# Wang-Xiaoyang/resource_packing_self_play

Hardware: AMD Instinct MI355X
Metric: self-play episodes/sec (with MCTS node expansions/sec alongside) (higher is better)
Workload: dtype f64 PUCT / f32 Q + CNN, u32 bit-board

## Files before the change

### resource_packing_self_play_amd/csrc/rp_engine.hip

```cpp
#include <hip/hip_runtime.h>
#include <math.h>
#include <stdarg.h>
#include <stdint.h>
#include <stdio.h>
#include <stdlib.h>
#include <string.h>

#include <algorithm>
#include <string>
#include <vector>

#include "../../include/rp_engine.h"

#pragma clang fp contract(off)

typedef unsigned long long u64;
typedef unsigned int u32;
typedef unsigned short u16;
typedef unsigned char u8;

#define NONE32 0xFFFFFFFFu
#define NSA_MASK 0x3FFFFFFFu
#define WAVES_PER_BLOCK 4
#define MAX_LEAVES 128
#define MAX_MASK_WORDS 256

enum { CNT_SIMS = 0, CNT_EXPAND, CNT_TERMINAL, CNT_PATH, CNT_NVALID_SEL, CNT_NVALID_LEAF, CNT_TRANSPOSE, CNT_NODES,
       CNT_MOVES, CNT_EPISODES, CNT_PROBES, CNT_KEYBYTES, CNT_VIS_SEL, CNT_VIS_NEW, CNT_RES0, CNT_RES1, CNT_N };
enum { ERR_NODE_CAP = 1, ERR_EDGE_CAP = 2, ERR_TABLE_FULL = 3, ERR_BAD_ACTION = 4, ERR_PATH = 5, ERR_FINISHED_CAP = 6, ERR_EXAMPLES_CAP = 7, ERR_VIS_CAP = 8, ERR_BAD_EXAMPLE = 9 };

struct NodeHdr {
    u32 ns;
    u32 prior_off;
    u32 vis_off;
    u16 n_valid;
    u16 vis_n;
    u16 vis_cap;
    int8_t term;
    u8 flags;
    u8 depth;
    u8 pad;
    u16 best_k;
    double norm;
};
#define HF_EXPANDED 1u
#define HF_FALLBACK 2u
__host__ __device__ inline u32 hdr_term_kind(const NodeHdr &h) { return (h.flags >> 2) & 3u; }

struct PoolDesc {
    long long n_instances;
    unsigned long long first_id;
    const unsigned char *wh;
    const int *area, *max_h;
    const unsigned long long *episode_id;
    const double *bl;
    const unsigned char *has_buf;
};
struct VisEntry {
    double q;
    double p;
    u32 n;
    u32 child;
    u32 idx;
    u32 pad;
};
struct DP {
    int W, H, N, A, G, sims, node_cap, edge_cap, vis_cap, table_cap, KW, RW, RMW, move_rule;
    int reclaim;
    int pchunk, n_pchunks, vchunk, n_vchunks;
    int step_cap;
    u32 magicW;
    double cpuct;
    u64 seed, tie_salt;
    u8 *item_wh;
    int *total_area, *max_h;
    double *bl;
    int *has_buf;
    u32 *root, *n_nodes;
    u16 *pa_cur, *pa_head, *pa_next, *pa_stack, *va_cur, *va_head, *va_next, *va_stack;
    u32 *pa_used, *pa_tf, *va_used, *va_tf;
    u32 *peak_chunks;
    int *phase, *sims_done, *moves;
    u64 *episode;
    u32 *leaf_node;
    int *path_len;
    u32 *path_edge, *path_node;
    int *game_row;
    int *last_outcome;
    double *last_score;
    double *last_v;
    int *last_vkind;
    int rows_identity;
// ... 2383 lines not shown
    for (int t = 0; t < NT; ++t) {
        const int m = t * 16 + n, pc = m < MP ? ptab[m] : IMGW * IMGP;
        abase[t] = (ptab[m < MP ? m : 0] - (PW + 1)) * PS + 8 * g;
        pdst[t][0] = pc * PS + 4 * g;
        pdst[t][1] = pc * PS + 16 + 4 * g;
    }
    const __amdgpu_buffer_rsrc_t frs = __builtin_amdgcn_make_buffer_rsrc((void *)frag, 0, 4 * 9 * CIN * 32 * 4, RS_BUF_FLAGS);
    constexpr int CONV_BYTES = 9 * CIN * 32 * 4;
    const int rowoff = n * 128 + g * 16;
    auto task_bytes = [&](long long l0) { return (int)(B - l0 < IMGW ? B - l0 : IMGW) * PIX * 128; };
    f32x4 xv[NT][2], xs[NT][2], wq[3][2];
    auto load_x = [&](long long l0) {
        const __amdgpu_buffer_rsrc_t rs = __builtin_amdgcn_make_buffer_rsrc((void *)(x + (size_t)l0 * PIX * CIN), 0, task_bytes(l0), RS_BUF_FLAGS);
#pragma unroll
        for (int t = 0; t < NT; ++t) { xv[t][0] = rs_load_x(rs, rowoff, t * 2048); xv[t][1] = rs_load_x(rs, rowoff, t * 2048 + 64); }
    };
    auto stage_x = [&]() {
#pragma unroll
        for (int t = 0; t < NT; ++t)
#pragma unroll
            for (int mt = 0; mt < 2; ++mt) { xs[t][mt] = xv[t][mt]; *(f32x4 *)(img + pdst[t][mt]) = rs_relu(xv[t][mt]); }
    };
    load_x(leaf0);
    wq[0][0] = rs_load_b(frs, lane * 16, 0); wq[0][1] = rs_load_b(frs, lane * 16, 1024);
    wq[1][0] = rs_load_b(frs, lane * 16, 2048); wq[1][1] = rs_load_b(frs, lane * 16, 3072);
    stage_x();
    if (leaf0 + stride_leaves < B) load_x(leaf0 + stride_leaves);
    for (; leaf0 < B; leaf0 += stride_leaves) {
        const int nbytes = task_bytes(leaf0);
        const __amdgpu_buffer_rsrc_t ors = __builtin_amdgcn_make_buffer_rsrc((void *)(out + (size_t)leaf0 * PIX * CIN), 0, nbytes, RS_BUF_FLAGS);
        f32x4 acc[NT][2];
#define R32_BIAS(k) const f32x4 ba = *(const f32x4 *)(sbias + 32 * (k) + 4 * g), bb = *(const f32x4 *)(sbias + 32 * (k) + 16 + 4 * g)
        lds_sync();
        r32_conv<NT, CIN>(img, frs, 0, CONV_BYTES, PW, abase, acc, wq);
        {
            R32_BIAS(0);
#pragma unroll
            for (int t = 0; t < NT; ++t) { *(f32x4 *)(img + pdst[t][0]) = rs_relu(acc[t][0] + ba); *(f32x4 *)(img + pdst[t][1]) = rs_relu(acc[t][1] + bb); }
        }
        lds_sync();
        r32_conv<NT, CIN>(img, frs, CONV_BYTES, 2 * CONV_BYTES, PW, abase, acc, wq);
        {
            R32_BIAS(1);
#pragma unroll
            for (int t = 0; t < NT; ++t) {
                xs[t][0] = (acc[t][0] + ba) + xs[t][0]; xs[t][1] = (acc[t][1] + bb) + xs[t][1];
                *(f32x4 *)(img + pdst[t][0]) = rs_relu(xs[t][0]); *(f32x4 *)(img + pdst[t][1]) = rs_relu(xs[t][1]);
            }
        }
        lds_sync();
        r32_conv<NT, CIN>(img, frs, 2 * CONV_BYTES, 3 * CONV_BYTES, PW, abase, acc, wq);
        {
            R32_BIAS(2);
#pragma unroll
            for (int t = 0; t < NT; ++t) { *(f32x4 *)(img + pdst[t][0]) = rs_relu(acc[t][0] + ba); *(f32x4 *)(img + pdst[t][1]) = rs_relu(acc[t][1] + bb); }
        }
        lds_sync();
        r32_conv<NT, CIN>(img, frs, 3 * CONV_BYTES, 0, PW, abase, acc, wq);
        {
            R32_BIAS(3);
#pragma unroll
            for (int t = 0; t < NT; ++t) {
                acc[t][0] = (acc[t][0] + ba) + xs[t][0]; acc[t][1] = (acc[t][1] + bb) + xs[t][1];
                __builtin_amdgcn_raw_buffer_store_b128(__builtin_bit_cast(u32x4, acc[t][0]), ors, rowoff, t * 2048, RS_STREAM_AUX);
                __builtin_amdgcn_raw_buffer_store_b128(__builtin_bit_cast(u32x4, acc[t][1]), ors, rowoff, t * 2048 + 64, RS_STREAM_AUX);
            }
        }
#undef R32_BIAS
        if (out_relu != nullptr) {
            const __amdgpu_buffer_rsrc_t rrs = __builtin_amdgcn_make_buffer_rsrc((void *)(out_relu + (size_t)leaf0 * PIX * CIN), 0, nbytes, RS_BUF_FLAGS);
#pragma unroll
            for (int t = 0; t < NT; ++t) {
                __builtin_amdgcn_raw_buffer_store_b128(__builtin_bit_cast(u32x4, rs_relu(acc[t][0])), rrs, rowoff, t * 2048, RS_STREAM_AUX);
                __builtin_amdgcn_raw_buffer_store_b128(__builtin_bit_cast(u32x4, rs_relu(acc[t][1])), rrs, rowoff, t * 2048 + 64, RS_STREAM_AUX);
            }
        }
        if (leaf0 + stride_leaves < B) {
            stage_x();
            if (leaf0 + 2 * stride_leaves < B) load_x(leaf0 + 2 * stride_leaves);
        }
    }
}

#define CP_PS 36
#ifdef CP_STAMP
__device__ unsigned long long g_cp_stamp[8];
#endif
template <int NT, int CIN, bool TAIL = false>
__global__ void __launch_bounds__(256, 2) k_convpool32(const float *__restrict__ x, const float *__restrict__ frag, const float *__restrict__ bias,
                                                       float *__restrict__ out, long long B, int S_h, int S_w, int IMGW, int wave_floats,
                                                       const int *__restrict__ nrows_dev) {
    constexpr int XQ = CIN / 16;
    constexpr int PS = CP_PS;
    extern __shared__ __attribute__((aligned(16))) float rb_lds[];
    const int lane = lane_id(), wv = wave_in_block();
    if (nrows_dev) { const long long n = *nrows_dev; if (n < B) B = n; }
    if (((long long)blockIdx.x * 4) * IMGW >= B) return;
    const int PW = r32_pw(S_w), PIX = S_h * S_w, IMGP = r32_imgp(S_h, S_w), MP = IMGW * PIX;
    const int Hp = (S_h + 1) >> 1, Wp = (S_w + 1) >> 1, PP = Hp * Wp;
    constexpr int NTT = NT + (TAIL ? 1 : 0);
    int *ptab = (int *)rb_lds;
    int *pool = ptab + 16 * NTT;
    float *img = rb_lds + 16 * NTT + ((IMGW * PP + 3) & ~3) + (size_t)wv * wave_floats;
    for (int i = threadIdx.x; i < 16 * NTT; i += blockDim.x) {
        int im = i / PIX, pq = i - im * PIX, r = pq / S_w, c = pq - r * S_w;
        ptab[i] = i < MP ? im * IMGP + (r + 1) * PW + c + 1 : 0;
    }
    for (int i = threadIdx.x; i < IMGW * PP; i += blockDim.x) {
        int im = i / PP, pp = i - im * PP, pr = pp / Wp, px = pp - pr * Wp;
        pool[i] = (im * IMGP + (2 * pr + 1) * PW + 2 * px + 1) | ((pr > 0) << 16) | ((2 * pr + 1 < S_h) << 17) | ((px > 0) << 18) | ((2 * px + 1 < S_w) << 19);
    }
    {
        float4 *z4 = (float4 *)img;
        for (int i = lane; i < wave_floats / 4; i += 64) z4[i] = make_float4(0.f, 0.f, 0.f, 0.f);
    }
    __syncthreads();
    const long long stride_leaves = (long long)gridDim.x * 4 * IMGW;
    long long leaf0 = ((long long)blockIdx.x * 4 + wv) * IMGW;
    if (leaf0 >= B) return;
    const int n = lane & 15, g = lane >> 4;
    int abase[NT], pin[NT];
#pragma unroll
    for (int t = 0; t < NT; ++t) {
        const int m = t * 16 + n, pc = m < MP ? ptab[m] : IMGW * IMGP;
        abase[t] = (ptab[m < MP ? m : 0] - (PW + 1)) * PS + CIN / 4 * g;
        pin[t] = pc * PS + 4 * g;
    }
    const __amdgpu_buffer_rsrc_t frs = __builtin_amdgcn_make_buffer_rsrc((void *)frag, 0, 9 * CIN * 32 * 4, RS_BUF_FLAGS);
    const f32x4 ba = *(const f32x4 *)(bias + 4 * g), bb = *(const f32x4 *)(bias + 16 + 4 * g);
    const int rowoff = n * (CIN * 4) + g * 16;
    auto task_bytes = [&](long long l0) { return (int)(B - l0 < IMGW ? B - l0 : IMGW) * PIX * CIN * 4; };
    f32x4 xv[NT][XQ], wq[3][2];
    int t_abase = 0, t_voff0 = 0, t_voff1 = 0;
    f32x4 t_acc = (f32x4){0.f, 0.f, 0.f, 0.f}, t_w0[2], t_w1[2];
    const int cg = lane >> 3, kk = (lane >> 2) & 1, mt = 16 * NT + (lane & 3);
    int pout_t = 0, pin_t = 0;
    f32x4 xvt = (f32x4){0.f, 0.f, 0.f, 0.f};
    const int xq_t = (lane >> 2) & (CIN / 4 - 1);
    const int rowoff_t = (lane & 3) * (CIN * 4) + xq_t * 16;
    if (TAIL) {
        const int pc = mt < MP ? ptab[mt] : IMGW * IMGP;
        t_abase = (ptab[mt < MP ? mt : 0] - (PW + 1)) * PS + (CIN / 2) * kk;
        const int lw = 4 * (cg & 3) + (lane & 3) + 32 * kk;
        t_voff0 = (cg >> 2) * 1024 + lw * 16; t_voff1 = (cg >> 2) * 1024 + (lw + 16) * 16;
        pout_t = pc * PS + 4 * cg;
        pin_t = pc * PS + 4 * xq_t;
    }
    auto load_x = [&](long long l0) {
        const __amdgpu_buffer_rsrc_t rs = __builtin_amdgcn_make_buffer_rsrc((void *)(x + (size_t)l0 * PIX * CIN), 0, task_bytes(l0), RS_BUF_FLAGS);
#pragma unroll
        for (int t = 0; t < NT; ++t)
#pragma unroll
            for (int q = 0; q < XQ; ++q) xv[t][q] = rs_load_x(rs, rowoff, t * 16 * CIN * 4 + 64 * q);
        if (TAIL) xvt = rs_load_x(rs, rowoff_t, NT * 16 * CIN * 4);
    };
    const int cq = lane & 7;
    load_x(leaf0);
    wq[0][0] = rs_load_b(frs, lane * 16, 0); wq[0][1] = rs_load_b(frs, lane * 16, 1024);
    wq[1][0] = rs_load_b(frs, lane * 16, 2048); wq[1][1] = rs_load_b(frs, lane * 16, 3072);
    if (TAIL) {
        t_w0[0] = rs_load_b(frs, t_voff0, 0); t_w1[0] = rs_load_b(frs, t_voff1, 0);
        t_w0[1] = rs_load_b(frs, t_voff0, 2048); t_w1[1] = rs_load_b(frs, t_voff1, 2048);
    }
#ifdef CP_STAMP
    unsigned long long st_acc[8] = {0, 0, 0, 0, 0, 0, 0, 0}, st_last = __builtin_amdgcn_s_memtime();
#define CP_T(k) { unsigned long long now_ = __builtin_amdgcn_s_memtime(); st_acc[k] += now_ - st_last; st_last = now_; }
// ... 289 lines not shown
        float4 *o4 = (float4 *)(out + (size_t)leaf0 * PP * 32);
        for (int pq = threadIdx.x >> 3; pq < nimg * PP; pq += 8 * WAVES) {
            const int im = pq / PP, pp = pq - im * PP, pr = pp / Wp, px = pp - pr * Wp;
            const int ctr = im * PIX + 2 * pr * S_w + 2 * px;
            const int ou = pr > 0 ? -S_w : 0, od = 2 * pr + 1 < S_h ? S_w : 0, ol = px > 0 ? -1 : 0, orr = 2 * px + 1 < S_w ? 1 : 0;
            const float4 *row = (const float4 *)(img + ctr * 36) + cq;
            const float4 v0 = row[0], v1 = row[ol * 9], v2 = row[orr * 9], v3 = row[ou * 9], v4 = row[(ou + ol) * 9], v5 = row[(ou + orr) * 9],
                         v6 = row[od * 9], v7 = row[(od + ol) * 9], v8 = row[(od + orr) * 9];
            float4 m;
            m.x = fmaxf(fmaxf(fmaxf(v0.x, v1.x), fmaxf(v2.x, v3.x)), fmaxf(fmaxf(v4.x, v5.x), fmaxf(fmaxf(v6.x, v7.x), v8.x)));
            m.y = fmaxf(fmaxf(fmaxf(v0.y, v1.y), fmaxf(v2.y, v3.y)), fmaxf(fmaxf(v4.y, v5.y), fmaxf(fmaxf(v6.y, v7.y), v8.y)));
            m.z = fmaxf(fmaxf(fmaxf(v0.z, v1.z), fmaxf(v2.z, v3.z)), fmaxf(fmaxf(v4.z, v5.z), fmaxf(fmaxf(v6.z, v7.z), v8.z)));
            m.w = fmaxf(fmaxf(fmaxf(v0.w, v1.w), fmaxf(v2.w, v3.w)), fmaxf(fmaxf(v4.w, v5.w), fmaxf(fmaxf(v6.w, v7.w), v8.w)));
            o4[pq * 8 + cq] = m;
        }
        lds_barrier();
        if (leaf0 + stride_leaves < B) {
            float4 *z4 = (float4 *)img;
            for (int i = threadIdx.x; i < wg_floats / 4; i += 64 * WAVES) z4[i] = make_float4(0.f, 0.f, 0.f, 0.f);
            lds_barrier();
        }
    }
}

struct rp_ctx {
    rp_config cfg;
    DP d;
    hipStream_t stream;
    bool row64;
    std::string err;
    std::vector<void *> allocs;
    int64_t bytes;
    int64_t fin_popped;
    u8 *pool_wh;
    int *pool_area, *pool_max_h;
    int64_t pool_cap;
    u64 *meta_id;
    double *meta_bl;
    u8 *meta_has;
    int64_t meta_cap;
    int n_cu = 256;
    size_t lds_per_cu = 160 * 1024;
    int compact_rows = 0;
    const int *nn_rows_dev = nullptr;
    u16 *tr_action = nullptr, *fin_tr_action = nullptr;
    u64 *tr_rows = nullptr, *fin_tr_rows = nullptr, *fin_board = nullptr;
};

static std::string g_create_error;

static int fail(rp_ctx *ctx, int code, const char *fmt, ...) {
    char buf[512];
    va_list ap;
    va_start(ap, fmt);
    vsnprintf(buf, sizeof buf, fmt, ap);
    va_end(ap);
    if (ctx) ctx->err = buf; else g_create_error = buf;
    return code;
}
#define HIPCHK(ctx, call)                                                                              \
    do {                                                                                               \
        hipError_t e_ = (call);                                                                        \
        if (e_ != hipSuccess) return fail(ctx, RP_ERR_DEVICE, "%s failed: %s", #call, hipGetErrorString(e_)); \
    } while (0)

template <typename T> static int dev_alloc(rp_ctx *ctx, T **out, size_t n, bool zero = true) {
    void *ptr = nullptr;
    size_t bytes = std::max<size_t>(n, 1) * sizeof(T);
    HIPCHK(ctx, hipMalloc(&ptr, bytes));
    ctx->allocs.push_back(ptr);
    ctx->bytes += (int64_t)bytes;
    if (zero) HIPCHK(ctx, hipMemsetAsync(ptr, 0, bytes, ctx->stream));
    *out = (T *)ptr;
    return RP_OK;
}
#define ALLOC(ctx, ptr, n)                       \
    do {                                         \
        int rc_ = dev_alloc(ctx, &(ptr), (n));   \
        if (rc_ != RP_OK) return rc_;            \
    } while (0)

#define STAGE_BYTES(d) ((size_t)WAVES_PER_BLOCK * (size_t)(d).A * sizeof(u16))

static int pick_leaves_per_wave(long long B, int PIX, int imgw_max) {
    const long long waves = 2048, typical = std::max<long long>(1, (long long)(0.92 * (double)B));
    long long best = -1;
    int pick = std::max(1, imgw_max);
    for (int k = std::max(1, imgw_max); k >= 1; --k) {
        const long long ntk = (k * PIX + 15) / 16;
        auto rounds = [&](long long rows) { const long long tasks = (rows + k - 1) / k; return (tasks + waves - 1) / waves; };
        const long long cost = (rounds(B) + 3 * rounds(typical)) * ntk;
        if (best < 0 || cost < best) { best = cost; pick = k; }
    }
    return pick;
}

static long long wg_group_cost(long long B, int k, int tile_slots, int n_cu) {
    const long long typical = std::max<long long>(1, (long long)(0.92 * (double)B));
    auto rounds = [&](long long rows) { const long long tasks = (rows + k - 1) / k; return (tasks + n_cu - 1) / n_cu; };
    return (rounds(B) + 3 * rounds(typical)) * tile_slots;
}

static int grid_for(long long waves) { return (int)((waves + WAVES_PER_BLOCK - 1) / WAVES_PER_BLOCK); }

static int allow_lds(rp_ctx *ctx, const void *fn, size_t lds, const char *what) {
    if (lds > ctx->lds_per_cu) return fail(ctx, RP_ERR_ARG, "%s: needs %zu bytes of LDS per workgroup, the device has %zu per CU", what, lds, ctx->lds_per_cu);
    if (lds <= 64 * 1024) return RP_OK;
    const hipError_t e = hipFuncSetAttribute(fn, hipFuncAttributeMaxDynamicSharedMemorySize, (int)lds);
    if (e != hipSuccess) return fail(ctx, RP_ERR_DEVICE, "%s: hipFuncSetAttribute(MaxDynamicSharedMemorySize = %zu) failed: %s", what, lds, hipGetErrorString(e));
    return RP_OK;
}

static int check_device_error(rp_ctx *ctx) {
    int e = 0;
    HIPCHK(ctx, hipMemcpyAsync(&e, ctx->d.error, sizeof(int), hipMemcpyDeviceToHost, ctx->stream));
    HIPCHK(ctx, hipStreamSynchronize(ctx->stream));
    if (e == 0) return RP_OK;
    (void)hipMemsetAsync(ctx->d.error, 0, sizeof(int), ctx->stream);
    static const char *names[] = {"", "node arena overflow (raise node_cap)", "legal-move arena overflow (raise edge_cap)",
                                  "transposition table full", "action is not a legal move of the (expanded) root", "search path broken",
                                  "finished-episode ring overflow", "replay buffer full (raise max_examples / max_sparse)",
                                  "visited-edge arena overflow (raise vis_cap)", "replay example index or sparse entry outside the packed arrays"};
    int code = (e == ERR_BAD_ACTION) ? RP_ERR_ASSERT : (e == ERR_PATH ? RP_ERR_STATE : (e == ERR_BAD_EXAMPLE ? RP_ERR_ARG : RP_ERR_CAPACITY));
    return fail(ctx, code, "device error %d: %s", e, e < 10 ? names[e] : "?");
}

static int build_plan(int lo, int n, std::vector<int> &llo, std::vector<int> &ln, std::vector<int> &sd, std::vector<int> &ss) {
    if (n <= 128) {
        llo.push_back(lo); ln.push_back(n);
        return (int)llo.size() - 1;
    }
    int n2 = n / 2;
    n2 -= n2 % 8;
    int a = build_plan(lo, n2, llo, ln, sd, ss);
    int b = build_plan(lo + n2, n - n2, llo, ln, sd, ss);
    sd.push_back(a); ss.push_back(b);
    return a;
}

extern "C" int rp_version(void) { return RP_ABI_VERSION; }

extern "C" const char *rp_last_error(const rp_ctx *ctx) { return ctx ? ctx->err.c_str() : g_create_error.c_str(); }

extern "C" int64_t rp_device_bytes(const rp_ctx *ctx) { return ctx ? ctx->bytes : 0; }

extern "C" void rp_destroy(rp_ctx *ctx) {
    if (!ctx) return;
    (void)hipSetDevice(ctx->cfg.device);
    (void)hipStreamSynchronize(ctx->stream);
    for (void *p : ctx->allocs) (void)hipFree(p);
    delete ctx;
}

extern "C" int rp_create(const rp_config *cfg, rp_ctx **out) {
    if (!cfg || !out) return fail(nullptr, RP_ERR_ARG, "null argument");
    *out = nullptr;
    if (cfg->abi_version != RP_ABI_VERSION) return fail(nullptr, RP_ERR_ARG, "abi_version %d != %d", cfg->abi_version, RP_ABI_VERSION);
    if (cfg->W < 1 || cfg->W > 64 || cfg->H < 1 || cfg->H > 64 || cfg->N < 1 || cfg->N > 128)
        return fail(nullptr, RP_ERR_ARG, "limits: 1<=W<=64, 1<=H<=64, 1<=N<=128 (got %d %d %d)", cfg->W, cfg->H, cfg->N);
    if (cfg->games < 1 || cfg->sims < 0) return fail(nullptr, RP_ERR_ARG, "games >= 1 and sims >= 0 required");
    if (!(cfg->cpuct > 0.0)) return fail(nullptr, RP_ERR_ARG, "cpuct must be positive (got %g): the best unvisited move of a node is kept as the one with the largest prior, which is the PUCT winner among the unvisited moves only for cpuct > 0", cfg->cpuct);
    if ((int64_t)cfg->sims * (cfg->N + 1) >= (int64_t)NSA_MASK) return fail(nullptr, RP_ERR_ARG, "sims too large");
    int ndev = 0;
    if (hipGetDeviceCount(&ndev) != hipSuccess || ndev <= cfg->device)
        return fail(nullptr, RP_ERR_DEVICE, "no HIP device %d (found %d): the engine has no CPU fallback", cfg->device, ndev);
    rp_ctx *ctx = new rp_ctx();
    ctx->cfg = *cfg;
    ctx->bytes = 0;
    ctx->fin_popped = 0;
    ctx->pool_wh = nullptr; ctx->pool_area = nullptr; ctx->pool_max_h = nullptr; ctx->pool_cap = 0;
    ctx->meta_id = nullptr; ctx->meta_bl = nullptr; ctx->meta_has = nullptr; ctx->meta_cap = 0;
    ctx->stream = (hipStream_t)cfg->stream;
    hipError_t e = hipSetDevice(cfg->device);
    if (e != hipSuccess) { delete ctx; return fail(nullptr, RP_ERR_DEVICE, "hipSetDevice: %s", hipGetErrorString(e)); }
    {
        hipDeviceProp_t prop;
        if (hipGetDeviceProperties(&prop, cfg->device) == hipSuccess) {
            if (prop.multiProcessorCount > 0) ctx->n_cu = prop.multiProcessorCount;
// ... 585 lines not shown
        }
#undef CPW_LAUNCH
        HIPCHK(ctx, hipGetLastError());
        return RP_OK;
    }
    const int PIX = H * W, max_tiles = Cin == 16 ? 7 : 5;
    const size_t img_pixels = (size_t)r32_imgp(H, W);
    int imgw = (16 * max_tiles) / PIX;
    const int PPn = ((H + 1) / 2) * ((W + 1) / 2);
    auto wave_floats = [&](int k) { return (size_t)(k * img_pixels + 1) * CP_PS; };
    auto lds_bytes = [&](int k) { return ((size_t)16 * ((k * PIX + 15) / 16) + (((size_t)k * PPn + 3) & ~(size_t)3) + 4 * wave_floats(k)) * sizeof(float); };
    while (imgw > 1 && lds_bytes(imgw) > 78 * 1024) --imgw;
    imgw = pick_leaves_per_wave(B, PIX, imgw);
    const int nt = (imgw * PIX + 15) / 16;
    const size_t wf = wave_floats(imgw), lds = lds_bytes(imgw);
    if (lds > ctx->lds_per_cu) return fail(ctx, RP_ERR_ARG, "rp_nn_convpool32: a %dx%d image needs %zu bytes of LDS per workgroup, the device has %zu per CU", H, W, lds, ctx->lds_per_cu);
    const long long tasks = (B + imgw - 1) / imgw;
    static const int cp_wgs = getenv("RP_CONVPOOL_WGS") ? atoi(getenv("RP_CONVPOOL_WGS")) : 2;
    const int per_cu = (int)std::max<size_t>(1, std::min<size_t>((size_t)cp_wgs, ctx->lds_per_cu / lds));
    const dim3 grid((unsigned)std::min<long long>((tasks + 3) / 4, (long long)ctx->n_cu * per_cu)), block(256);
#define CP_LAUNCH(NT_, CIN_)                                                                                                                         \
    {                                                                                                                                                \
        const int rc_ = allow_lds(ctx, (const void *)k_convpool32<NT_, CIN_>, lds, "rp_nn_convpool32"); if (rc_ != RP_OK) return rc_;                \
        hipLaunchKernelGGL((k_convpool32<NT_, CIN_>), grid, block, lds, ctx->stream, x_dev, frag_dev, bias_dev, out_dev, (long long)B, (int)H,        \
                           (int)W, imgw, (int)wf, ctx->nn_rows_dev);                                                                                 \
    }
    static const int cp_tail = getenv("RP_CONVPOOL_TAIL") ? atoi(getenv("RP_CONVPOOL_TAIL")) : 1;
    const int tail_px = (imgw * PIX) & 15;
    if (cp_tail && Cin == 16 && nt == 7 && tail_px >= 1 && tail_px <= 4) {
        const int rc_ = allow_lds(ctx, (const void *)k_convpool32<6, 16, true>, lds, "rp_nn_convpool32"); if (rc_ != RP_OK) return rc_;
        hipLaunchKernelGGL((k_convpool32<6, 16, true>), grid, block, lds, ctx->stream, x_dev, frag_dev, bias_dev, out_dev, (long long)B, (int)H, (int)W, imgw, (int)wf, ctx->nn_rows_dev);
    } else if (Cin == 16) {
        switch (nt) {
            case 1: CP_LAUNCH(1, 16) break; case 2: CP_LAUNCH(2, 16) break; case 3: CP_LAUNCH(3, 16) break; case 4: CP_LAUNCH(4, 16) break;
            case 5: CP_LAUNCH(5, 16) break; case 6: CP_LAUNCH(6, 16) break; case 7: CP_LAUNCH(7, 16) break;
            default: return fail(ctx, RP_ERR_ARG, "rp_nn_convpool32: unsupported image size");
        }
    } else {
        switch (nt) {
            case 1: CP_LAUNCH(1, 32) break; case 2: CP_LAUNCH(2, 32) break; case 3: CP_LAUNCH(3, 32) break; case 4: CP_LAUNCH(4, 32) break;
            case 5: CP_LAUNCH(5, 32) break;
            default: return fail(ctx, RP_ERR_ARG, "rp_nn_convpool32: unsupported image size");
        }
    }
#undef CP_LAUNCH
    HIPCHK(ctx, hipGetLastError());
    return RP_OK;
}

extern "C" int rp_nn_resstage32(rp_ctx *ctx, const float *x_dev, const float *frag4_dev, const float *bias4_dev, float *out_dev, float *out_relu_dev, int64_t B,
                                int32_t H, int32_t W) {
    if (!ctx || !x_dev || !frag4_dev || !bias4_dev || !out_dev || B < 0 || H < 1 || W < 1 || H * W > 512)
        return fail(ctx, RP_ERR_ARG, "rp_nn_resstage32: bad argument (images of at most 512 pixels)");
    if (B == 0) return RP_OK;
    const int PIX = H * W;
    if (PIX > 80) {
        const size_t img_px = (size_t)r32_imgp(H, W);
        auto lds_of = [&](int k) { return (128 + (k * img_px + 1) * r32_ps(32)) * sizeof(float); };
        int imgw = 1, nt = 0, waves = 4;
        long long best = -1;
        for (int k = 1; k * PIX <= 512 && lds_of(k) <= ctx->lds_per_cu; ++k) {
            const int tk = (k * PIX + 15) / 16, wk = tk > 16 ? 8 : 4, ntk = (tk + wk - 1) / wk;
            const long long cost = wg_group_cost(B, k, wk * ntk, ctx->n_cu);
            if (best < 0 || cost < best) { best = cost; imgw = k; nt = ntk; waves = wk; }
        }
        if (nt == 0) return fail(ctx, RP_ERR_ARG, "rp_nn_resstage32: a %dx%d image does not fit LDS", H, W);
        const size_t lds = lds_of(imgw);
        const long long tasks = (B + imgw - 1) / imgw;
        const int per_cu = (int)std::max<size_t>(1, std::min<size_t>(2, ctx->lds_per_cu / lds));
        const dim3 grid((unsigned)std::min<long long>(tasks, (long long)ctx->n_cu * per_cu)), block(64 * waves);
#define RSW_LAUNCH(NT_, WV_)                                                                                                                        \
    case NT_ * 16 + WV_: {                                                                                                                          \
        const int rc_ = allow_lds(ctx, (const void *)k_resstage32_wg<NT_, WV_>, lds, "rp_nn_resstage32"); if (rc_ != RP_OK) return rc_;            \
        hipLaunchKernelGGL((k_resstage32_wg<NT_, WV_>), grid, block, lds, ctx->stream, x_dev, frag4_dev, bias4_dev, out_dev, out_relu_dev, (long long)B, (int)H, (int)W, imgw, ctx->nn_rows_dev); \
    } break;
        switch (nt * 16 + waves) {
            RSW_LAUNCH(2, 4) RSW_LAUNCH(3, 4) RSW_LAUNCH(4, 4) RSW_LAUNCH(3, 8) RSW_LAUNCH(4, 8)
            default: return fail(ctx, RP_ERR_ARG, "rp_nn_resstage32: unsupported image size");
        }
#undef RSW_LAUNCH
        HIPCHK(ctx, hipGetLastError());
        return RP_OK;
    }
    const size_t img_pixels = (size_t)r32_imgp(H, W);
    auto lds_bytes = [&](int k) { return ((size_t)16 * ((k * PIX + 15) / 16) + 128 + 4 * (k * img_pixels + 1) * r32_ps(32)) * sizeof(float); };
    int imgw_max = 80 / PIX;
    while (imgw_max > 1 && lds_bytes(imgw_max) > 78 * 1024) --imgw_max;
    const int imgw = pick_leaves_per_wave(B, PIX, imgw_max);
    const int nt = (imgw * PIX + 15) / 16;
    const size_t lds = lds_bytes(imgw);
    if (lds > ctx->lds_per_cu) return fail(ctx, RP_ERR_ARG, "rp_nn_resstage32: a %dx%d image needs %zu bytes of LDS per workgroup, the device has %zu per CU", H, W, lds, ctx->lds_per_cu);
    const long long tasks = (B + imgw - 1) / imgw;
    static const int rs32_wgs = getenv("RP_STAGE32_WGS") ? atoi(getenv("RP_STAGE32_WGS")) : 2;
    const int per_cu = (int)std::max<size_t>(1, std::min<size_t>((size_t)rs32_wgs, ctx->lds_per_cu / lds));
    const dim3 grid((unsigned)std::min<long long>((tasks + 3) / 4, (long long)ctx->n_cu * per_cu)), block(256);
#define RS_LAUNCH(NT_)                                                                                                                              \
    case NT_:                                                                                                                                       \
        { const int rc_ = allow_lds(ctx, (const void *)k_resstage32<NT_>, lds, "rp_nn_resstage32"); if (rc_ != RP_OK) return rc_; }                \
        hipLaunchKernelGGL(k_resstage32<NT_>, grid, block, lds, ctx->stream, x_dev, frag4_dev, bias4_dev, out_dev, out_relu_dev,                    \
                           (long long)B, (int)H, (int)W, imgw, ctx->nn_rows_dev);                                                                   \
        break;
    switch (nt) {
        RS_LAUNCH(1) RS_LAUNCH(2) RS_LAUNCH(3) RS_LAUNCH(4) RS_LAUNCH(5)
        default: return fail(ctx, RP_ERR_ARG, "rp_nn_resstage32: unsupported image size");
    }
#undef RS_LAUNCH
    HIPCHK(ctx, hipGetLastError());
    return RP_OK;
}

extern "C" int rp_leaf_states(rp_ctx *ctx, int32_t max_rows, uint64_t *rows_out, uint8_t *remaining_out, int32_t *slot_out, int32_t *n_out) {
    if (!ctx || max_rows < 0 || !rows_out || !remaining_out || !slot_out || !n_out) return fail(ctx, RP_ERR_ARG, "rp_leaf_states: bad argument");
    const DP &d = ctx->d;
    if (d.rows_identity) return fail(ctx, RP_ERR_STATE, "rp_leaf_states: call rp_search_step with n_leaves_out first (compact rows)");
    int n = 0;
    HIPCHK(ctx, hipMemcpyAsync(&n, d.eval_count, sizeof(int), hipMemcpyDeviceToHost, ctx->stream));
    HIPCHK(ctx, hipStreamSynchronize(ctx->stream));
    n = std::min(n, (int)max_rows);
    *n_out = n;
    if (n == 0) return RP_OK;
    Scratch s(ctx);
    u64 *drows = s.up((const u64 *)nullptr, (size_t)n * d.H); NEED(drows);
    u8 *drem = s.up((const u8 *)nullptr, (size_t)n * d.N); NEED(drem);
    int *dslot = s.up((const int *)nullptr, (size_t)n); NEED(dslot);
    DISPATCH(ctx, k_leaf_states, grid_for(n), d, drows, drem, dslot, n);
    HIPCHK(ctx, hipMemcpyAsync(rows_out, drows, (size_t)n * d.H * 8, hipMemcpyDeviceToHost, ctx->stream));
    HIPCHK(ctx, hipMemcpyAsync(remaining_out, drem, (size_t)n * d.N, hipMemcpyDeviceToHost, ctx->stream));
    HIPCHK(ctx, hipMemcpyAsync(slot_out, dslot, (size_t)n * sizeof(int), hipMemcpyDeviceToHost, ctx->stream));
    HIPCHK(ctx, hipStreamSynchronize(ctx->stream));
    return RP_OK;
}

static int launch_commit(rp_ctx *ctx, const float *pi_dev, const float *v_dev, bool logits) {
    const DP &d = ctx->d;
    const dim3 grid(grid_for(d.G)), block(64 * WAVES_PER_BLOCK);
    const size_t lds = (size_t)WAVES_PER_BLOCK * ((size_t)d.n_leaves * sizeof(double) + (size_t)std::min(d.A, TERM_CHUNK) * sizeof(float) +
                                                 (logits ? (size_t)d.A * sizeof(float) : 0) + (size_t)(((d.A + 31) >> 5) + 1) * sizeof(u32));
    if (logits) {
        if (ctx->row64) hipLaunchKernelGGL((k_commit<u64, true>), grid, block, lds, ctx->stream, d, pi_dev, v_dev);
        else hipLaunchKernelGGL((k_commit<u32, true>), grid, block, lds, ctx->stream, d, pi_dev, v_dev);
    } else {
        if (ctx->row64) hipLaunchKernelGGL((k_commit<u64, false>), grid, block, lds, ctx->stream, d, pi_dev, v_dev);
        else hipLaunchKernelGGL((k_commit<u32, false>), grid, block, lds, ctx->stream, d, pi_dev, v_dev);
    }
    hipError_t le_ = hipGetLastError();
    if (le_ != hipSuccess) return fail(ctx, RP_ERR_DEVICE, "launch of k_commit failed: %s", hipGetErrorString(le_));
    return RP_OK;
}

extern "C" int rp_commit_eval(rp_ctx *ctx, const float *pi_dev, const float *v_dev) {
    if (!ctx || !pi_dev || !v_dev) return fail(ctx, RP_ERR_ARG, "rp_commit_eval: bad argument");
    return launch_commit(ctx, pi_dev, v_dev, false);
}

extern "C" int rp_commit_eval_logits(rp_ctx *ctx, const float *logits_dev, const float *v_dev) {
    if (!ctx || !logits_dev || !v_dev) return fail(ctx, RP_ERR_ARG, "rp_commit_eval_logits: bad argument");
    if ((size_t)WAVES_PER_BLOCK * ctx->d.A * sizeof(float) > 24 * 1024)
        return fail(ctx, RP_ERR_ARG, "rp_commit_eval_logits: %d actions do not fit the kernel's LDS row buffers (at most 1536): take the softmax first and call rp_commit_eval", ctx->d.A);
    return launch_commit(ctx, logits_dev, v_dev, true);
}

extern "C" int rp_commit_eval_host(rp_ctx *ctx, const float *pi_host, const float *v_host, int32_t n_rows) {
    if (!ctx || !pi_host || !v_host || n_rows < 0) return fail(ctx, RP_ERR_ARG, "rp_commit_eval_host: bad argument");
    const DP &d = ctx->d;
    if (d.rows_identity) return fail(ctx, RP_ERR_STATE, "rp_commit_eval_host: call rp_search_step with n_leaves_out first (compact rows)");
    int n = 0;
    HIPCHK(ctx, hipMemcpyAsync(&n, d.eval_count, sizeof(int), hipMemcpyDeviceToHost, ctx->stream));
    HIPCHK(ctx, hipStreamSynchronize(ctx->stream));
    if (n_rows < n) return fail(ctx, RP_ERR_ARG, "rp_commit_eval_host: %d rows given, %d leaves waiting", n_rows, n);
    if (n == 0) return RP_OK;
    Scratch s(ctx);
    float *dpi = s.up(pi_host, (size_t)n * d.A); NEED(dpi);
    float *dv = s.up(v_host, (size_t)n); NEED(dv);
    { const int rc = launch_commit(ctx, dpi, dv, false); if (rc != RP_OK) return rc; }
    HIPCHK(ctx, hipStreamSynchronize(ctx->stream));
    return check_device_error(ctx);
// ... 427 lines not shown
```

Before: 1394.

## Add position-major resstage32 kernel for 3x3 and 5x5 boards with cost-based dispatch

Adds a new residual-stage kernel that maps 16 leaves to the MFMA N dimension and walks compile-time tables of (position, tap) pairs, so only valid 3x3 conv taps are computed instead of padded pixel tiles. For 5x5 boards the 25 positions are split across four waves that share one LDS image; for 3x3 each wave owns its own image. A host cost model compares it with the existing pixel-tiled path and picks one, with an env override. The tables are fully unrolled, which raises register pressure, and the 5x5 variant needs block-wide barriers between stages.

After: 1537, median of 6. 10.3% higher.

```diff
diff --git a/resource_packing_self_play_amd/csrc/rp_engine.hip b/resource_packing_self_play_amd/csrc/rp_engine.hip
--- a/resource_packing_self_play_amd/csrc/rp_engine.hip
+++ b/resource_packing_self_play_amd/csrc/rp_engine.hip
@@ -8,6 +8,7 @@
 
 #include <algorithm>
 #include <string>
+#include <utility>
 #include <vector>
 
 #include "../../include/rp_engine.h"
@@ -2557,6 +2558,169 @@
     }
 }
 
+__host__ __device__ constexpr int pm_swz(int n) { return (((n >> 1) & 1) | (((n >> 2) & 1) * 6)) ^ ((n & 1) * 4); }
+__host__ __device__ constexpr int pm_in_pos(int S, int p, int tap) {
+    const int r = p / S + tap / 3 - 1, c = p % S + tap % 3 - 1;
+    return (r >= 0 && r < S && c >= 0 && c < S) ? r * S + c : -1;
+}
+__host__ __device__ constexpr int pm_role_pos(int S, int role, int i) {
+    if (S == 3) return i < 9 ? i : -1;
+    constexpr int t[4][8] = {{6, 7, 11, 12, 1, -1, -1, -1}, {8, 13, 17, 18, 23, -1, -1, -1}, {16, 2, 3, 5, 9, 10, 0, -1}, {14, 15, 19, 21, 22, 4, 20, 24}};
+    return i < 8 ? t[role][i] : -1;
+}
+struct PmList {
+    int n, np, ok;
+    int pos[9];
+    signed char s[100], k[100], q[100];
+};
+constexpr PmList pm_make_list(int S, int role) {
+    PmList L{};
+    while (L.np < 9 && pm_role_pos(S, role, L.np) >= 0) { L.pos[L.np] = pm_role_pos(S, role, L.np); ++L.np; }
+    L.ok = 1;
+    for (int s = 0; s < 18; ++s) {
+        int cnt = 0;
+        for (int k = 0; k < L.np; ++k) {
+            const int q = pm_in_pos(S, L.pos[k], s / 2);
+            if (q < 0) continue;
+            L.s[L.n] = (signed char)s; L.k[L.n] = (signed char)k; L.q[L.n] = (signed char)q; ++L.n; ++cnt;
+        }
+        if (cnt == 0) L.ok = 0;
+    }
+    return L;
+}
+template <int S, int ROLE> struct PmTab { static constexpr PmList L = pm_make_list(S, ROLE); };
+static_assert(PmTab<3, 0>::L.n == 98 && PmTab<3, 0>::L.ok, "3x3: 49 (position, tap) pairs");
+static_assert(PmTab<5, 0>::L.n + PmTab<5, 1>::L.n + PmTab<5, 2>::L.n + PmTab<5, 3>::L.n == 2 * 169 && PmTab<5, 0>::L.np + PmTab<5, 1>::L.np + PmTab<5, 2>::L.np + PmTab<5, 3>::L.np == 25 &&
+              PmTab<5, 0>::L.ok && PmTab<5, 1>::L.ok && PmTab<5, 2>::L.ok && PmTab<5, 3>::L.ok, "5x5: 169 pairs over four waves");
+template <class F, int... I> __device__ __forceinline__ void pm_for_(F &&f, std::integer_sequence<int, I...>) { (f(std::integral_constant<int, I>{}), ...); }
+template <int N, class F> __device__ __forceinline__ void pm_for(F &&f) { pm_for_(f, std::make_integer_sequence<int, N>{}); }
+template <int S> __device__ __forceinline__ void pm_sync() {
+    if constexpr (S == 3) lds_sync(); else lds_barrier();
+}
+#define PM_IMG_FLOATS(S) ((S) * (S) * 16 * 32)
+template <int S, int ROLE>
+__device__ __forceinline__ void pm_body(const float *__restrict__ x, const float *__restrict__ frag, float *__restrict__ out, float *__restrict__ out_relu, long long B,
+                                        long long leaf0, long long stride_leaves, const float *sbias, float *img) {
+    using T = PmTab<S, ROLE>;
+    constexpr int NP = T::L.np, NE = T::L.n, PIX = S * S, CONV_BYTES = 9 * 32 * 32 * 4;
+    const int lane = lane_id(), n = lane & 15, g = lane >> 4, sw = pm_swz(n);
+    const float *rb0 = img + n * 32 + 4 * ((2 * g) ^ sw), *rb1 = img + n * 32 + 4 * ((2 * g + 1) ^ sw);
+    float *wb0 = img + n * 32 + 4 * (g ^ sw), *wb1 = img + n * 32 + 4 * ((4 + g) ^ sw);
+    const int voff = lane * 16, xoff = n * (PIX * 128) + g * 16;
+    const __amdgpu_buffer_rsrc_t frs = __builtin_amdgcn_make_buffer_rsrc((void *)frag, 0, 4 * CONV_BYTES, RS_BUF_FLAGS);
+    f32x4 xs[NP][2], acc[NP][2], wq[3][2], bq[3];
+    wq[0][0] = rs_load_b(frs, voff, 0); wq[0][1] = rs_load_b(frs, voff, 1024);
+    wq[1][0] = rs_load_b(frs, voff, 2048); wq[1][1] = rs_load_b(frs, voff, 3072);
+    auto b_read = [&](auto E) {
+        constexpr int e = decltype(E)::value, off = T::L.q[e] * 512;
+        return *(const f32x4 *)(((T::L.s[e] & 1) ? rb1 : rb0) + off);
+    };
+    for (; leaf0 < B; leaf0 += stride_leaves) {
+        const int nbytes = (int)(B - leaf0 < 16 ? B - leaf0 : 16) * PIX * 128;
+        const __amdgpu_buffer_rsrc_t xrs = __builtin_amdgcn_make_buffer_rsrc((void *)(x + (size_t)leaf0 * PIX * 32), 0, nbytes, RS_BUF_FLAGS);
+        pm_for<NP>([&](auto K) {
+            constexpr int k = decltype(K)::value, p = T::L.pos[k];
+            xs[k][0] = rs_load_x(xrs, xoff, p * 128); xs[k][1] = rs_load_x(xrs, xoff, p * 128 + 64);
+        });
+        pm_for<NP>([&](auto K) {
+            constexpr int k = decltype(K)::value, p = T::L.pos[k];
+            *(f32x4 *)(wb0 + p * 512) = rs_relu(xs[k][0]); *(f32x4 *)(wb1 + p * 512) = rs_relu(xs[k][1]);
+            __builtin_amdgcn_sched_barrier(0);
+        });
+        pm_sync<S>();
+#pragma unroll 1
+        for (int kc = 0; kc < 4; ++kc) {
+            const int fbase = kc * CONV_BYTES, fnext = ((kc + 1) & 3) * CONV_BYTES;
+            pm_for<NP>([&](auto K) {
+                constexpr int k = decltype(K)::value;
+                acc[k][0] = (f32x4){0.f, 0.f, 0.f, 0.f}; acc[k][1] = (f32x4){0.f, 0.f, 0.f, 0.f};
+            });
+            bq[0] = b_read(std::integral_constant<int, 0>{}); bq[1] = b_read(std::integral_constant<int, 1>{});
+            pm_for<NE>([&](auto E) {
+                constexpr int e = decltype(E)::value, s = T::L.s[e], k = T::L.k[e];
+                if constexpr (e == 0 || T::L.s[e > 0 ? e - 1 : 0] != s) {
+                    constexpr int s2 = s + 2;
+                    const int off = s2 < 18 ? fbase + s2 * 2048 : fnext + (s2 - 18) * 2048;
+                    wq[s2 % 3][0] = rs_load_b(frs, voff, off); wq[s2 % 3][1] = rs_load_b(frs, voff, off + 1024);
+                }
+                if constexpr (e + 2 < NE) bq[(e + 2) % 3] = b_read(std::integral_constant<int, (e + 2 < NE ? e + 2 : 0)>{});
+                const f32x4 w0 = wq[s % 3][0], w1 = wq[s % 3][1], b = bq[e % 3];
+                __builtin_amdgcn_sched_barrier(0);
+#pragma unroll
+                for (int j = 0; j < 4; ++j) {
+                    acc[k][0] = __builtin_amdgcn_mfma_f32_16x16x4f32(w0[j], b[j], acc[k][0], 0, 0, 0);
+                    acc[k][1] = __builtin_amdgcn_mfma_f32_16x16x4f32(w1[j], b[j], acc[k][1], 0, 0, 0);
+                }
+                __builtin_amdgcn_sched_barrier(0);
+            });
+            pm_sync<S>();
+            const f32x4 ba = *(const f32x4 *)(sbias + 32 * kc + 4 * g), bb = *(const f32x4 *)(sbias + 32 * kc + 16 + 4 * g);
+            if (kc < 3) {
+                if (kc == 1)
+                    pm_for<NP>([&](auto K) {
+                        constexpr int k = decltype(K)::value, p = T::L.pos[k];
+                        xs[k][0] = (acc[k][0] + ba) + xs[k][0]; xs[k][1] = (acc[k][1] + bb) + xs[k][1];
+                        *(f32x4 *)(wb0 + p * 512) = rs_relu(xs[k][0]); *(f32x4 *)(wb1 + p * 512) = rs_relu(xs[k][1]);
+                        __builtin_amdgcn_sched_barrier(0);
+                    });
+                else
+                    pm_for<NP>([&](auto K) {
+                        constexpr int k = decltype(K)::value, p = T::L.pos[k];
+                        *(f32x4 *)(wb0 + p * 512) = rs_relu(acc[k][0] + ba); *(f32x4 *)(wb1 + p * 512) = rs_relu(acc[k][1] + bb);
+                        __builtin_amdgcn_sched_barrier(0);
+                    });
+                pm_sync<S>();
+            } else {
+                const __amdgpu_buffer_rsrc_t ors = __builtin_amdgcn_make_buffer_rsrc((void *)(out + (size_t)leaf0 * PIX * 32), 0, nbytes, RS_BUF_FLAGS);
+                pm_for<NP>([&](auto K) {
+                    constexpr int k = decltype(K)::value, p = T::L.pos[k];
+                    acc[k][0] = (acc[k][0] + ba) + xs[k][0]; acc[k][1] = (acc[k][1] + bb) + xs[k][1];
+                    __builtin_amdgcn_raw_buffer_store_b128(__builtin_bit_cast(u32x4, acc[k][0]), ors, xoff, p * 128, RS_STREAM_AUX);
+                    __builtin_amdgcn_raw_buffer_store_b128(__builtin_bit_cast(u32x4, acc[k][1]), ors, xoff, p * 128 + 64, RS_STREAM_AUX);
+                    __builtin_amdgcn_sched_barrier(0);
+                });
+                if (out_relu != nullptr) {
+                    const __amdgpu_buffer_rsrc_t rrs = __builtin_amdgcn_make_buffer_rsrc((void *)(out_relu + (size_t)leaf0 * PIX * 32), 0, nbytes, RS_BUF_FLAGS);
+                    pm_for<NP>([&](auto K) {
+                        constexpr int k = decltype(K)::value, p = T::L.pos[k];
+                        __builtin_amdgcn_raw_buffer_store_b128(__builtin_bit_cast(u32x4, rs_relu(acc[k][0])), rrs, xoff, p * 128, RS_STREAM_AUX);
+                        __builtin_amdgcn_raw_buffer_store_b128(__builtin_bit_cast(u32x4, rs_relu(acc[k][1])), rrs, xoff, p * 128 + 64, RS_STREAM_AUX);
+                        __builtin_amdgcn_sched_barrier(0);
+                    });
+                }
+            }
+        }
+    }
+}
+template <int S>
+__global__ void __launch_bounds__(256, 2) k_resstage32_pm(const float *__restrict__ x, const float *__restrict__ frag, const float *__restrict__ bias,
+                                                          float *__restrict__ out, float *__restrict__ out_relu, long long B, const int *__restrict__ nrows_dev) {
+    extern __shared__ __attribute__((aligned(16))) float rb_lds[];
+    const int wv = wave_in_block();
+    if (nrows_dev) { const long long n = *nrows_dev; if (n < B) B = n; }
+    float *sbias = rb_lds;
+    if constexpr (S == 3) {
+        if ((long long)blockIdx.x * 64 >= B) return;
+        for (int i = threadIdx.x; i < 128; i += blockDim.x) sbias[i] = bias[i];
+        __syncthreads();
+        const long long leaf0 = ((long long)blockIdx.x * 4 + wv) * 16;
+        if (leaf0 >= B) return;
+        pm_body<3, 0>(x, frag, out, out_relu, B, leaf0, (long long)gridDim.x * 64, sbias, rb_lds + 128 + (size_t)wv * PM_IMG_FLOATS(3));
+    } else {
+        if ((long long)blockIdx.x * 16 >= B) return;
+        for (int i = threadIdx.x; i < 128; i += blockDim.x) sbias[i] = bias[i];
+        __syncthreads();
+        const long long leaf0 = (long long)blockIdx.x * 16, stride = (long long)gridDim.x * 16;
+        float *img = rb_lds + 128;
+        switch (wv) {
+            case 0: pm_body<5, 0>(x, frag, out, out_relu, B, leaf0, stride, sbias, img); break;
+            case 1: pm_body<5, 1>(x, frag, out, out_relu, B, leaf0, stride, sbias, img); break;
+            case 2: pm_body<5, 2>(x, frag, out, out_relu, B, leaf0, stride, sbias, img); break;
+            default: pm_body<5, 3>(x, frag, out, out_relu, B, leaf0, stride, sbias, img); break;
+        }
+    }
+}
+
 #define CP_PS 36
 #ifdef CP_STAMP
 __device__ unsigned long long g_cp_stamp[8];
@@ -3012,8 +3176,9 @@
 
 #define STAGE_BYTES(d) ((size_t)WAVES_PER_BLOCK * (size_t)(d).A * sizeof(u16))
 
+#define STAGE_WAVES 2048
 static int pick_leaves_per_wave(long long B, int PIX, int imgw_max) {
-    const long long waves = 2048, typical = std::max<long long>(1, (long long)(0.92 * (double)B));
+    const long long waves = STAGE_WAVES, typical = std::max<long long>(1, (long long)(0.92 * (double)B));
     long long best = -1;
     int pick = std::max(1, imgw_max);
     for (int k = std::max(1, imgw_max); k >= 1; --k) {
@@ -3024,6 +3189,30 @@
     }
     return pick;
 }
+
+static long long pm_rounds_cost(long long B, int k, long long units) {
+    const long long typical = std::max<long long>(1, (long long)(0.92 * (double)B));
+    auto rounds = [&](long long rows) { const long long tasks = (rows + k - 1) / k; return (tasks + units - 1) / units; };
+    return rounds(B) + 3 * rounds(typical);
+}
+static size_t r32_wave_lds(int H, int W, int k) { return ((size_t)16 * ((k * H * W + 15) / 16) + 128 + 4 * ((size_t)k * r32_imgp(H, W) + 1) * r32_ps(32)) * sizeof(float); }
+static void r32_wave_plan(long long B, int H, int W, int *imgw, int *nt) {
+    const int PIX = H * W;
+    int imgw_max = 80 / PIX;
+    while (imgw_max > 1 && r32_wave_lds(H, W, imgw_max) > 78 * 1024) --imgw_max;
+    *imgw = pick_leaves_per_wave(B, PIX, imgw_max);
+    *nt = (*imgw * PIX + 15) / 16;
+}
+static bool stage32_pm_cheaper(long long B, int H, int W) {
+    if (H != W || (H != 3 && H != 5) || B <= 0) return false;
+    int imgw, nt;
+    r32_wave_plan(B, H, W, &imgw, &nt);
+    const long long cost_old = pm_rounds_cost(B, imgw, STAGE_WAVES) * nt * 9;
+    const long long cost_pm = H == 3 ? pm_rounds_cost(B, 16, STAGE_WAVES) * 49 : pm_rounds_cost(B, 16, STAGE_WAVES / 4) * 43;
+    return cost_pm < cost_old;
+}
+extern "C" int rp_debug_stage32_pm_pick(int64_t B, int32_t H, int32_t W) { return stage32_pm_cheaper(B, H, W) ? 1 : 0; }
+extern "C" int rp_debug_stage32_pm_swz(int32_t n) { return pm_swz(n); }
 
 static long long wg_group_cost(long long B, int k, int tile_slots, int n_cu) {
     const long long typical = std::max<long long>(1, (long long)(0.92 * (double)B));
@@ -3775,16 +3964,31 @@
         HIPCHK(ctx, hipGetLastError());
         return RP_OK;
     }
-    const size_t img_pixels = (size_t)r32_imgp(H, W);
-    auto lds_bytes = [&](int k) { return ((size_t)16 * ((k * PIX + 15) / 16) + 128 + 4 * (k * img_pixels + 1) * r32_ps(32)) * sizeof(float); };
-    int imgw_max = 80 / PIX;
-    while (imgw_max > 1 && lds_bytes(imgw_max) > 78 * 1024) --imgw_max;
-    const int imgw = pick_leaves_per_wave(B, PIX, imgw_max);
-    const int nt = (imgw * PIX + 15) / 16;
-    const size_t lds = lds_bytes(imgw);
+    int imgw, nt;
+    r32_wave_plan(B, H, W, &imgw, &nt);
+    static const int rs32_wgs = getenv("RP_STAGE32_WGS") ? atoi(getenv("RP_STAGE32_WGS")) : 2;
+    if (H == W && (H == 3 || H == 5)) {
+        const char *pm_env = getenv("RP_STAGE32_PM");
+        const int pm_force = pm_env ? atoi(pm_env) : -1;
+        if (pm_force == 1 || (pm_force != 0 && stage32_pm_cheaper(B, H, W))) {
+            const size_t lds_pm = (128 + (size_t)(H == 3 ? 4 : 1) * PM_IMG_FLOATS(H)) * sizeof(float);
+            const long long tasks_pm = (B + 15) / 16, wgs = H == 3 ? (tasks_pm + 3) / 4 : tasks_pm;
+            const int per_cu_pm = (int)std::max<size_t>(1, std::min<size_t>((size_t)rs32_wgs, ctx->lds_per_cu / lds_pm));
+            const dim3 grid_pm((unsigned)std::min<long long>(wgs, (long long)ctx->n_cu * per_cu_pm)), block_pm(256);
+            if (H == 3) {
+                const int rc_ = allow_lds(ctx, (const void *)k_resstage32_pm<3>, lds_pm, "rp_nn_resstage32"); if (rc_ != RP_OK) return rc_;
+                hipLaunchKernelGGL(k_resstage32_pm<3>, grid_pm, block_pm, lds_pm, ctx->stream, x_dev, frag4_dev, bias4_dev, out_dev, out_relu_dev, (long long)B, ctx->nn_rows_dev);
+            } else {
+                const int rc_ = allow_lds(ctx, (const void *)k_resstage32_pm<5>, lds_pm, "rp_nn_resstage32"); if (rc_ != RP_OK) return rc_;
+                hipLaunchKernelGGL(k_resstage32_pm<5>, grid_pm, block_pm, lds_pm, ctx->stream, x_dev, frag4_dev, bias4_dev, out_dev, out_relu_dev, (long long)B, ctx->nn_rows_dev);
+            }
+            HIPCHK(ctx, hipGetLastError());
+            return RP_OK;
+        }
+    }
+    const size_t lds = r32_wave_lds(H, W, imgw);
     if (lds > ctx->lds_per_cu) return fail(ctx, RP_ERR_ARG, "rp_nn_resstage32: a %dx%d image needs %zu bytes of LDS per workgroup, the device has %zu per CU", H, W, lds, ctx->lds_per_cu);
     const long long tasks = (B + imgw - 1) / imgw;
-    static const int rs32_wgs = getenv("RP_STAGE32_WGS") ? atoi(getenv("RP_STAGE32_WGS")) : 2;
     const int per_cu = (int)std::max<size_t>(1, std::min<size_t>((size_t)rs32_wgs, ctx->lds_per_cu / lds));
     const dim3 grid((unsigned)std::min<long long>((tasks + 3) / 4, (long long)ctx->n_cu * per_cu)), block(256);
 #define RS_LAUNCH(NT_)                                                                                                                              \
```
